# lizaibeim/mmla-audio

Hardware: AMD Instinct MI355X
Metric: audio clips/sec (MFCC→logits) at 1/2/4/8 MI355X; MFCC max-abs-err vs librosa (higher is better)
Workload: dtype f16x3+f32

## Files before the change

mmla_audio_amd/csrc/context.cpp:

```cpp
#include <algorithm>
#include <cstdarg>
#include <cstdio>
#include <cstdlib>

#include "internal.h"

using namespace mmla;

namespace mmla __attribute__((visibility("hidden"))) {

int fail(mmla_ctx* c, int code, const char* fmt, ...) {
  char buf[512];
  va_list ap;
  va_start(ap, fmt);
  vsnprintf(buf, sizeof(buf), fmt, ap);
  va_end(ap);
  if (c) c->err = buf;
  return code;
}

static hipEvent_t prof_event(mmla_ctx* c) {
  if (!c->prof_pool.empty()) {
    hipEvent_t e = c->prof_pool.back();
    c->prof_pool.pop_back();
// ... 77 lines not shown
  return MMLA_OK;
}

int ws_release(mmla_ctx* c) {
  HIPCHK(c, hipStreamSynchronize(c->stream));
  for (size_t i = 0; i < c->ws.size(); ++i)
    if (c->ws[i]) {
      HIPCHK(c, hipFree(static_cast<char*>(c->ws[i]) - c->ws_guard[i]));
      c->ws[i] = nullptr;
      c->ws_size[i] = 0;
      c->ws_guard[i] = 0;
    }
  return MMLA_OK;
}

static int ws_check_guards(mmla_ctx* c) {
  std::vector<unsigned char> h(kGuardBytes);
  for (size_t slot = 0; slot < c->ws.size(); ++slot) {
    const size_t g = c->ws_guard[slot];
    if (!c->ws[slot] || !g) continue;
    for (int side = 0; side < 2; ++side) {
      const char* d = static_cast<const char*>(c->ws[slot]) + (side ? c->ws_size[slot] : -(ptrdiff_t)g);
      HIPCHK(c, hipMemcpy(h.data(), d, g, hipMemcpyDeviceToHost));
      for (size_t i = 0; i < g; ++i)
        if (h[i] != kGuardByte)
          return fail(c, MMLA_E_HIP, "workspace slot %zu: %s guard overwritten at byte %zu", slot,
                      side ? "trailing" : "leading", side ? i : g - i);
    }
  }
  return MMLA_OK;
}

int finish(mmla_ctx* c, bool dev) {
  HIPCHK(c, hipGetLastError());
  bool guarded = false;
  for (size_t g : c->ws_guard) guarded |= g != 0;
  if (!dev || guarded) HIPCHK(c, hipStreamSynchronize(c->stream));
  if (guarded) return ws_check_guards(c);
  return MMLA_OK;
}

constexpr double kOdBytesPerClip = 3.0 * 128 * 151 * 32 * 4 + 128 * 151 * 3 + 128 * 151 * 4 +
                                   19 * 128 * 4 + 512 * 4 + 64;
constexpr double kSiBytesPerClip = 4.0 * 256 * 32 * 4 + 256 * 39 * 4 + 8 * 128 * 4 + 512 * 4 +
                                   1024 * 4 + 64;

int64_t microbatch(mmla_ctx* c, bool od) {
  const int64_t user = od ? c->od_mb : c->si_mb;
  if (user > 0) return user;
  const int64_t cap = od ? c->od_mb_cap : c->si_mb_cap;
  size_t fr = 0, tot = 0;
  if (hipMemGetInfo(&fr, &tot) != hipSuccess) {
    (void)hipGetLastError();
    return cap;
  }
  double held = 0;
  for (size_t b : c->ws_size) held += (double)b;
  int64_t fit = (int64_t)(((double)fr + held) * 0.9 / (od ? kOdBytesPerClip : kSiBytesPerClip));
  fit = fit / kMinMicrobatch * kMinMicrobatch;
  return std::max(kMinMicrobatch, std::min(cap, fit));
}

}

struct EnvSwitch {
  const char* name;
  bool mmla_ctx::*no;
  int mmla_ctx::*num;
};
static const EnvSwitch kEnvSwitches[] = {
    {"MMLA_DEBUG_FAIL_ALLOC", nullptr, &mmla_ctx::debug_fail_allocs},
    {"MMLA_NO_SIU", &mmla_ctx::siu, nullptr},
    {"MMLA_NO_SIPU", &mmla_ctx::sipu, nullptr},
    {"MMLA_NO_SIFIN", &mmla_ctx::sifin, nullptr},
    {"MMLA_NO_SIPAIR", &mmla_ctx::sipair, nullptr},
    {"MMLA_NO_SICHAIN", &mmla_ctx::sichain, nullptr},
    {"MMLA_NO_LSTM_SPLIT", &mmla_ctx::lstm_split, nullptr},
    {"MMLA_LSTM_SPLIT_MAX", nullptr, &mmla_ctx::lstm_split_max},
    {"MMLA_DEBUG_LSTM_SPIN", nullptr, &mmla_ctx::lstm_spin},
    {"MMLA_NO_SIPAD", &mmla_ctx::si_pad_feat, nullptr},
    {"MMLA_NO_ODU", &mmla_ctx::odu, nullptr},
    {"MMLA_NO_ODW", &mmla_ctx::odw, nullptr},
    {"MMLA_RB_TILE", &mmla_ctx::rbs, nullptr},
    {"MMLA_NO_PIN_OUT", &mmla_ctx::pin_small, nullptr},
};

extern "C" {

int mmla_abi_version(void) { return MMLA_ABI_VERSION; }

int mmla_create(int device, mmla_ctx** out) {
  if (!out) return MMLA_E_INVALID;
  *out = nullptr;
  int ndev = 0;
  if (hipGetDeviceCount(&ndev) != hipSuccess || ndev == 0) return MMLA_E_HIP;
  if (device < 0 || device >= ndev) return MMLA_E_INVALID;
  if (hipSetDevice(device) != hipSuccess) return MMLA_E_HIP;
  mmla_ctx* c = new mmla_ctx();
  c->device = device;
  for (const EnvSwitch& s : kEnvSwitches)
    if (const char* v = std::getenv(s.name)) {
      if (s.no) c->*s.no = std::atoi(v) == 0;
      else c->*s.num = std::atoi(v);
    }
  if (hipStreamCreateWithFlags(&c->own_stream, hipStreamDefault) != hipSuccess) {
    delete c;
    return MMLA_E_HIP;
  }
  c->stream = c->own_stream;
  if (hipMalloc(&c->range_dev, 4 * sizeof(int)) != hipSuccess ||
      hipMemset(c->range_dev, 0, 4 * sizeof(int)) != hipSuccess ||
      hipHostMalloc(&c->range_host, 2 * sizeof(int), hipHostMallocDefault) != hipSuccess) {
    mmla_destroy(c);
    return MMLA_E_HIP;
  }
  if (c->pin_small) {
    const unsigned fl = hipHostMallocMapped | hipHostMallocCoherent;
    if (hipHostMalloc(reinterpret_cast<void**>(&c->range_map), 64, fl) != hipSuccess ||
        hipHostGetDevicePointer(reinterpret_cast<void**>(&c->range_map_dev), c->range_map, 0) != hipSuccess ||
        hipHostMalloc(reinterpret_cast<void**>(&c->pin_out), kPinSlots * kPinSlotBytes, fl) != hipSuccess ||
        hipHostGetDevicePointer(reinterpret_cast<void**>(&c->pin_out_dev), c->pin_out, 0) != hipSuccess ||
        hipHostMalloc(reinterpret_cast<void**>(&c->pin_in), kPinInBytes, hipHostMallocDefault) != hipSuccess) {
      mmla_destroy(c);
      return MMLA_E_HIP;
    }
    c->range_map[0] = c->range_map[1] = 0;
  }
  OdFeTables ot;
  od_fe_build_tables(&ot);
  if (!od_fe_tables_ok(ot)) {
    mmla_destroy(c);
    return MMLA_E_INVALID;
  }
  SiFeTables st;
  si_fe_build_tables(&st);
  if (!si_fe_tables_ok(st)) {
    mmla_destroy(c);
    return MMLA_E_INVALID;
  }
  if (hipMalloc(&c->od_tables, sizeof(OdFeTables)) != hipSuccess ||
      hipMalloc(&c->si_tables, sizeof(SiFeTables)) != hipSuccess ||
      hipMemcpy(c->od_tables, &ot, sizeof(ot), hipMemcpyHostToDevice) != hipSuccess ||
      hipMemcpy(c->si_tables, &st, sizeof(st), hipMemcpyHostToDevice) != hipSuccess) {
    mmla_destroy(c);
    return MMLA_E_HIP;
  }
  *out = c;
  return MMLA_OK;
}

int mmla_destroy(mmla_ctx* c) {
  if (!c) return MMLA_E_INVALID;
  (void)hipSetDevice(c->device);
  if (c->stream) (void)hipStreamSynchronize(c->stream);
  free_allocs(c->od_allocs);
  free_allocs(c->si_allocs);
  for (size_t i = 0; i < c->ws.size(); ++i)
    if (c->ws[i]) (void)hipFree(static_cast<char*>(c->ws[i]) - c->ws_guard[i]);
  if (c->od_tables) (void)hipFree(c->od_tables);
  if (c->si_tables) (void)hipFree(c->si_tables);
  if (c->nr_tables) (void)hipFree(c->nr_tables);
  if (c->nr_thresh) (void)hipFree(c->nr_thresh);
  if (c->range_dev) (void)hipFree(c->range_dev);
  if (c->vad_state) (void)hipFree(c->vad_state);
  if (c->range_host) (void)hipHostFree(c->range_host);
  if (c->range_map) (void)hipHostFree(c->range_map);
// ... 120 lines not shown
```

mmla_audio_amd/csrc/internal.h:

```cpp
#pragma once
#include <hip/hip_runtime.h>

#include <cstdint>
#include <cstring>
#include <string>
#include <vector>

#include "../../include/mmla.h"
#include "nr.h"
#include "od_fe.h"
#include "si_fe.h"
#include "ssim.h"
#include "vad.h"

namespace mmla __attribute__((visibility("hidden"))) {

constexpr int OD_H = 128, OD_W = 151, OD_PIX = OD_H * OD_W;
constexpr int OD_IMG = OD_PIX * 3;
constexpr int SI_T = 256, SI_D = 39;
constexpr int SI_NEED_SAMPLES = 160 * 259 + 400;
constexpr int CH[9] = {32, 32, 32, 64, 64, 64, 128, 128, 128};
constexpr bool POOL[9] = {true, false, false, true, false, false, true, false, false};

struct ConvW {
// ... 8 lines not shown
  float unscale() const { return 1.0f / (16.0f * wscale); }
};
struct BnW {
  float* scale = nullptr;
  float* shift = nullptr;
  int c = 0;
};
struct LstmW {
  float* wcat[2] = {nullptr, nullptr};
  float* bias[2] = {nullptr, nullptr};
  uint16_t* wth[2] = {nullptr, nullptr};
  uint16_t* wtl[2] = {nullptr, nullptr};
  float ws[2] = {256.0f, 256.0f};
};
struct ResUnitW {
  BnW bn_in, bn_mid;
  ConvW ca, cb, sc;
};
struct OdNet {
  ConvW stem;
  ResUnitW blk[9];
  LstmW lstm;
  float* head_w = nullptr;
  float* head_b = nullptr;
};
struct SiNet {
  ConvW stem;
  ResUnitW unit[9];
  BnW final_bn;
  LstmW lstm;
  ConvW dense;
  int k = 0, head = 0;
};

struct ProfRec {
  int stage;
  hipEvent_t a, b;
  double work;
};

constexpr int64_t kOdMicrobatch = 16384;
constexpr int64_t kSiMicrobatch = 65536;
constexpr int64_t kMinMicrobatch = 64;

constexpr size_t kPinSlotBytes = 64u << 10;
constexpr size_t kPinInBytes = 1u << 20;
constexpr int kPinSlots = 4;

}

struct mmla_ctx {
  bool prof_on = false;
  std::vector<mmla::ProfRec> prof_pending;
  std::vector<hipEvent_t> prof_pool;
  double prof_ms[MMLA_NSTAGES] = {0};
  double prof_work[MMLA_NSTAGES] = {0};
  int64_t prof_n[MMLA_NSTAGES] = {0};
  int device = 0;
  hipStream_t stream = nullptr;
  hipStream_t own_stream = nullptr;
  std::string err;
  OdFeTables* od_tables = nullptr;
  SiFeTables* si_tables = nullptr;
  bool od_loaded = false, si_loaded = false;
  mmla::OdNet od;
  mmla::SiNet si;
  std::vector<void*> od_allocs, si_allocs;
  std::vector<void*> ws;
  std::vector<size_t> ws_size;
  std::vector<size_t> ws_guard;
  int64_t od_mb = 0, si_mb = 0;
  int64_t od_mb_cap = mmla::kOdMicrobatch, si_mb_cap = mmla::kSiMicrobatch;
  int debug_fail_allocs = 0;
  int precision = MMLA_PREC_F16X3;
  bool siu = true;
  bool sipu = true;
  bool sifin = true;
  bool sipair = true;
  bool sichain = true;
  bool si_pad_feat = true;
  bool odu = true;
  bool odw = true;
  bool rbs = true;
  bool lstm_split = true;
  int lstm_split_max = 128;
  int lstm_spin = 0;
  int* range_dev = nullptr;
  int* range_host = nullptr;
  bool pin_small = true;
  int* range_map = nullptr;
  int* range_map_dev = nullptr;
  char* pin_out = nullptr;
  char* pin_out_dev = nullptr;
  char* pin_in = nullptr;
  int* range_ptr = nullptr;
  int* timeout_ptr = nullptr;
  int64_t lstm_split_reruns = 0;
  int64_t range_reruns = 0;
  bool od_f32_only = false, si_f32_only = false;
  bool loading_f16_bad = false;
  VadState* vad_state = nullptr;
  int64_t vad_streams = 0;
  NrTables* nr_tables = nullptr;
  float* nr_thresh = nullptr;
  int64_t nr_profiles = 0;
  bool nr_ready = false;
};

namespace mmla __attribute__((visibility("hidden"))) {

int fail(mmla_ctx* c, int code, const char* fmt, ...);

#define HIPCHK(ctx, expr)                                                                        \
  do {                                                                                           \
    hipError_t e_ = (expr);                                                                      \
    if (e_ != hipSuccess)                                                                        \
      return mmla::fail(ctx, MMLA_E_HIP, "%s failed: %s (%s:%d)", #expr, hipGetErrorString(e_), \
                        __FILE__, __LINE__);                                                     \
  } while (0)

#define CHK(expr)              \
  do {                         \
    int r_ = (expr);           \
    if (r_ != MMLA_OK) return r_; \
  } while (0)

int prof_begin(mmla_ctx* c, int stage);
void prof_end(mmla_ctx* c, int idx, double work);
int prof_collect(mmla_ctx* c);

#define LAUNCH(c, st, wk, expr)                  \
  do {                                           \
    const int pi_ = mmla::prof_begin((c), (st)); \
    HIPCHK((c), (expr));                         \
    mmla::prof_end((c), pi_, (wk));              \
  } while (0)

enum Slot {
  S_PCM = 0, S_LENS, S_IMG, S_X, S_T1, S_T2, S_T3, S_SEQ, S_HOUT, S_LOGIT, S_FEAT, S_SILENT,
  S_OUT0, S_OUT1, S_OUT2, S_OUT3, S_IN,
  S_NR_S, S_NR_BITS, S_NR_FMAX, S_NR_FRAMES, S_NR_ITEMS, S_NR_Y, S_NR_ROWS,
  S_VAD_SPEECH, S_VAD_OUT, S_VAD_LENS, S_RS_TR, S_RS_WIN, S_LSTM,
  S_TRAIN,
  S_IMG2, S_GATE_Y0, S_GATE_Y1, S_SSIM,
  S_NR_PROF, S_COND_Q, S_COND_KEPT
};

int ws_get(mmla_ctx* c, int slot, size_t bytes, void** out);
int ws_release(mmla_ctx* c);
int64_t microbatch(mmla_ctx* c, bool od);
int finish(mmla_ctx* c, bool dev);
void free_allocs(std::vector<void*>& al);
int nr_reduce_dev(mmla_ctx* c, const float* y, int64_t n_signals, int64_t stride, int64_t len, float* out,
                  const int32_t* profile = nullptr);

template <typename T>
int in_ptr(mmla_ctx* c, const T* user, size_t count, bool dev, int slot, const T** d) {
  *d = user;
  if (dev || !user) return MMLA_OK;
  void* p = nullptr;
  CHK(ws_get(c, slot, count * sizeof(T), &p));
  HIPCHK(c, hipMemcpyAsync(p, user, count * sizeof(T), hipMemcpyHostToDevice, c->stream));
  *d = static_cast<const T*>(p);
  return MMLA_OK;
}

// ... 51 lines not shown
```

mmla_audio_amd/csrc/net_runners.cpp:

```cpp
#include <algorithm>

#include "conv.h"
#include "conv_h3.h"
#include "internal.h"
#include "nets.h"
#include "odu.h"
#include "resblk.h"
#include "siu.h"

using namespace mmla;

namespace {

ConvArgs conv_args(const ConvW& w, const float* x, float* y, int n, int h, int wd, int stride,
                   const BnW* bn, int pro, int epi, const float* res) {
  ConvArgs a{};
  a.x = x;
  a.wt = w.wt;
  a.bias = w.bias;
  a.scale = bn ? bn->scale : nullptr;
  a.shift = bn ? bn->shift : nullptr;
  a.res = res;
  a.y = y;
  a.n = n;
// ... 208 lines not shown
  o.s_in = B.bn_in.scale;
  o.t_in = B.bn_in.shift;
  o.s_mid = B.bn_mid.scale;
  o.t_mid = B.bn_mid.shift;
  o.ua = B.ca.unscale();
  o.ub = B.cb.unscale();
  o.n = (int)n;
  o.range_flag = range_flag;
  if (pool) {
    o.wsh = B.sc.wh;
    o.wsl = B.sc.wl;
    o.bs = B.sc.bias;
    o.us = B.sc.unscale();
  }
  return o;
}

double od_block_flops(const ResUnitW& B, bool pool, int64_t n, int h, int w) {
  return 2.0 * n * h * w * (9.0 * B.ca.cin * B.ca.cout + 4.0 * B.cb.cin * B.cb.cout) +
         (pool ? 2.0 * n * ((h + 1) / 2) * ((w + 1) / 2) * B.sc.cin * B.sc.cout : 0.0);
}

int od_block_pair(mmla_ctx* c, const ResUnitW& B, bool pool, int n, int h, int w, float* X, float*& T1,
                  float*& T2, float** out) {
  CHK(conv_spatial(c, B.ca, X, T1, n, h, w, &B.bn_in, PRO_BN_ELU, EPI_BIAS, nullptr));
  if (!pool) {
    *out = X;
    return conv_spatial(c, B.cb, T1, X, n, h, w, &B.bn_mid, PRO_BN_ELU, EPI_ADD, X);
  }
  if (c->precision != MMLA_PREC_F16X3) {
    CHK(conv_spatial(c, B.cb, T1, T2, n, h, w, &B.bn_mid, PRO_BN_ELU, EPI_BIAS, nullptr));
    ConvArgs s = conv_args(B.sc, X, T1, n, h, w, 2, nullptr, PRO_NONE, EPI_ADD_POOL, T2);
    s.hp = h;
    s.wp = w;
    CHK(conv_run(c, s));
  } else if (B.sc.wh && B.sc.cout == B.cb.cout && B.cb.cout_pad == B.sc.cout_pad) {
    CHK(conv_spatial(c, B.cb, T1, T2, n, h, w, &B.bn_mid, PRO_BN_ELU, EPI_BIAS, nullptr, true, 0, &B.sc,
                     X));
    std::swap(T1, T2);
  } else {
    CHK(conv_spatial(c, B.cb, T1, T2, n, h, w, &B.bn_mid, PRO_BN_ELU, EPI_BIAS, nullptr, true));
    CHK(conv_run(c, conv_args(B.sc, X, T1, n, h, w, 2, nullptr, PRO_NONE, EPI_ADD, T2)));
  }
  *out = T1;
  return MMLA_OK;
}

}

namespace mmla __attribute__((visibility("hidden"))) {

int run_od_net(mmla_ctx* c, const uint8_t* img_u8, const float* img_f32, int64_t n, float* probs,
               int32_t* argmax, OdGate gate, int stop, const float** tap, int64_t* tap_n) {
  const OdNet& W = c->od;
  const size_t big = (size_t)n * OD_PIX * 32;
  float *X, *T1, *T2, *SEQ, *H;
  CHK(ws_floats(c, S_X, big, &X));
  CHK(ws_floats(c, S_T1, big, &T1));
  CHK(ws_floats(c, S_T2, big, &T2));
  CHK(ws_floats(c, S_SEQ, (size_t)n * 19 * 128, &SEQ));
  CHK(ws_floats(c, S_HOUT, (size_t)n * 512, &H));
  const double stem_flops = 2.0 * n * OD_PIX * 3 * 16;
  const OdChoice first = od_choose(c, W.blk[0], 0, OD_H, OD_W, stop);
  if (!first.stem)
    LAUNCH(c, MMLA_STAGE_GLUE, stem_flops,
           od_stem_launch(img_u8, img_f32, n * OD_PIX, W.stem.cout_pad, W.stem.wt, W.stem.bias, X,
                          c->stream));
  int h = OD_H, w = OD_W;
  if (stop == 0) {
    *tap = X;
    *tap_n = n * OD_PIX * 16;
    return MMLA_OK;
  }
  for (int b = 0; b < 9; ++b) {
    const ResUnitW& B = W.blk[b];
    const bool pool = POOL[b];
    const OdChoice k = b == 0 ? first : od_choose(c, B, b, h, w, stop);
    const double flops = od_block_flops(B, pool, n, h, w) + (k.stem ? stem_flops : 0.0);
    float* out = T1;
    switch (k.path) {
      case OD_STRIPS:
      case OD_TILES: {
        const bool tiles = k.path == OD_TILES;
        const ResBlkArgs r = resblk_args(B, pool, tiles, X, T1, n, h, w, c->range_ptr,
                                         k.stem ? &W.stem : nullptr, img_u8, img_f32);
        LAUNCH(c, MMLA_STAGE_CONV, flops,
               tiles ? resblk_launch(r, B.ca.cin, B.ca.cout, pool, c->stream)
                     : rbs_launch(r, B.ca.cin, B.ca.cout, pool, c->stream));
        break;
      }
      case OD_ODU: {
        const OduArgs o = odu_args(B, pool, X, T1, n, c->range_ptr);
        LAUNCH(c, MMLA_STAGE_CONV, flops,
               odu_launch(o, h, w, B.ca.cin, B.ca.cout, pool, k.strips, c->stream));
        break;
      }
      case OD_PAIR:
        CHK(od_block_pair(c, B, pool, (int)n, h, w, X, T1, T2, &out));
        break;
    }
    if (pool) {
      h = (h + 1) / 2;
      w = (w + 1) / 2;
    }
    if (out != X) std::swap(X, T1);
    if (stop == b + 1) {
      *tap = X;
      *tap_n = n * h * w * CH[b];
      return MMLA_OK;
    }
  }
  LAUNCH(c, MMLA_STAGE_GLUE, (double)n * h * w * 128,
         mean_h_launch(X, (int)n, h, w, 128, SEQ, c->stream));
  if (stop == 10) {
    *tap = SEQ;
    *tap_n = n * w * 128;
    return MMLA_OK;
  }
  LAUNCH(c, MMLA_STAGE_LSTM, lstm_flops(n, w, 128),
         lstm_run(c, W.lstm, SEQ, n, w, H));
  if (stop == 11) {
    *tap = H;
    *tap_n = n * 512;
    return MMLA_OK;
  }
  LAUNCH(c, MMLA_STAGE_HEAD, 2.0 * n * 512 * 2,
         od_head_launch(H, (int)n, W.head_w, W.head_b, probs, argmax,
                        gate.lens, gate.clip_len, gate.silent, gate.ssim, gate.ssim_threshold,
                        c->stream));
  return MMLA_OK;
}

}


namespace {

bool siu_ok(const ResUnitW& U, int cin) {
  return U.ca.wh && U.cb.wh && siu_supported(cin) && U.ca.cin == cin && U.ca.cout == cin && U.cb.cin == cin &&
         U.cb.cout == cin && U.ca.cin_pad == cin && U.ca.cout_pad == cin && U.cb.cout_pad == cin;
}

bool sipu_ok(const ResUnitW& U, int cin) {
  return U.ca.wh && U.cb.wh && U.sc.wh && sipu_supported(cin, U.ca.cout) && U.ca.cin_pad == cin &&
         U.ca.cout_pad == U.ca.cout && U.cb.cin == U.ca.cout && U.cb.cout == U.ca.cout &&
         U.cb.cout_pad == U.ca.cout && U.sc.cin == cin && U.sc.cout == U.ca.cout &&
         U.sc.cout_pad == U.ca.cout;
}

SiuArgs siu_args(const ResUnitW& U, const float* x, float* y, int64_t n, int t, int* range_flag,
                 int t_src = 0) {
  SiuArgs s{};
  s.n = (int)n;
  s.t = t;
  s.range_flag = range_flag;
  s.x = x;
  s.y = y;
  s.wah = U.ca.wh;
  s.wal = U.ca.wl;
  s.wbh = U.cb.wh;
  s.wbl = U.cb.wl;
  s.ba = U.ca.bias;
  s.bb = U.cb.bias;
  s.s_in = U.bn_in.scale;
  s.t_in = U.bn_in.shift;
  s.s_mid = U.bn_mid.scale;
  s.t_mid = U.bn_mid.shift;
  s.ua = U.ca.unscale();
// ... 130 lines not shown
```

mmla_audio_amd/csrc/rbs.hip:

```cpp
#include "f16x3.h"
#include "resblk.h"

namespace {

constexpr int NT = 256;
constexpr int TW = 16;
constexpr int R = 8;
constexpr int C = 32;
#ifndef RBS_TRACE
#define RBS_TRACE 0
#endif
#if RBS_TRACE
__device__ unsigned long long rbs_trace_buf[2048 * 4 * 4 * 8];
#define RBS_T(i) do { if (bid < 2048 && k >= 2 && k < 6) tt[i] = __builtin_amdgcn_s_memtime(); } while (0)
#define RBS_TFLUSH() do { if (bid < 2048 && k >= 2 && k < 6 && lane == 0) { for (int i_ = 0; i_ < 8; ++i_) rbs_trace_buf[(((size_t)bid * 4 + wave) * 4 + (k - 2)) * 8 + i_] = tt[i_]; } } while (0)
#else
#define RBS_T(i) do { } while (0)
#define RBS_TFLUSH() do { } while (0)
#endif

template <int H, int W, int CIN, bool POOL>
struct SG {
  static constexpr int XW = TW + 2;
  static constexpr int XRING = R + 2, TRING = R + 3;
  static constexpr int XROW = XW * CIN;
  static constexpr int XPLANE = XRING * XROW;
  static constexpr int TROW = TW * C;
  static constexpr int TPLANE = TRING * TROW;
  static constexpr int NCHUNK = H / R;
  static constexpr int STRIPS = (W + TW - 1) / TW;
  static constexpr int QPP = CIN / 4;
  static constexpr int MAXT = (R * XW * QPP + NT - 1) / NT;
  static constexpr int MAXT0 = (4 * XW * QPP + NT - 1) / NT;
  static constexpr int KPT = CIN / 16;
  static constexpr int KS1 = 9 * KPT, KS2 = 8;
  static constexpr bool W2L = CIN == 16;
  static constexpr int MINB = CIN == 16 ? 3 : 2;
  static constexpr int PF = 3;
  static constexpr int PD = CIN == 16 ? 1 : 2;
  static_assert(H % R == 0, "geometry");
  static_assert(NT % QPP == 0, "a thread's channel quad is fixed");
  static_assert(XROW <= 1024 && W * CIN * 4 < 65536 && W * 12 < 65536, "staging task fields");
};

template <int CIN>
MMLA_DEV int xoff(int slot, int x, int g) {
  constexpr int XROW = (TW + 2) * CIN;
  const int f = CIN == 32 ? ((x >> 1) & 3) : ((x >> 1) & 1);
  return slot * XROW + x * CIN + 8 * (g ^ f);
}
template <bool POOL>
MMLA_DEV int toff(int slot, int j, int c, int g) {
  const int f = POOL ? (((c >> 2) ^ (2 * (j & 1))) & 3) : ((c >> 2) & 3);
  return slot * (TW * C) + c * C + 8 * (g ^ f);
}

template <int H, int W, int CIN, bool POOL, bool STEM>
__global__ void __launch_bounds__(NT, (SG<H, W, CIN, POOL>::MINB)) rbs_kernel(ResBlkArgs a) {
  using G = SG<H, W, CIN, POOL>;
  static_assert(!STEM || (CIN == 16 && POOL), "the stem feeds block 1");
  static_assert(POOL || CIN == C, "residual blocks keep their width");
  __shared__ __attribute__((aligned(16))) _Float16 sx[2 * G::XPLANE];
  __shared__ __attribute__((aligned(16))) _Float16 st[2 * G::TPLANE];
  __shared__ float4 spar[3 * C / 4 + (STEM ? 16 : 0)];
  __shared__ __attribute__((aligned(16))) _Float16 sw2[G::W2L ? 2 * G::KS2 * 512 : 8];

  const int tid = threadIdx.x, lane = tid & 63;
  const int wave = __builtin_amdgcn_readfirstlane(tid >> 6);
  const int h = lane >> 5;
  const uint32_t bid = xcd_block_id();
  const int clip = (int)(bid / G::STRIPS);
  const int w0 = (int)(bid - (uint32_t)clip * G::STRIPS) * TW;
  const int lofs = lane * 8;
  float rmax = 0.0f;

  float* const sp = reinterpret_cast<float*>(spar);
  if (tid < C) {
    const float s2 = a.s2[tid];
    sp[tid] = 16.0f * (s2 * a.u1);
    sp[C + tid] = 16.0f * fmaf(a.b1[tid], s2, a.t2[tid]);
    sp[2 * C + tid] = a.b2[tid];
  }
  if constexpr (STEM) {
    if (tid < 64) {
      const int co = tid >> 2, k = tid & 3;
      sp[3 * C + tid] = k < 3 ? a.wst[k * a.ldst + co] : a.bst[co];
    }
  }
  const __amdgpu_buffer_rsrc_t rw1h = w_rsrc(a.w1h), rw1l = w_rsrc(a.w1l);
  f16x8 w2h[G::W2L ? 1 : G::KS2], w2l[G::W2L ? 1 : G::KS2];
  if constexpr (G::W2L) {
    for (int e = tid; e < 2 * G::KS2 * 64; e += NT) {
      const int pl = e / (G::KS2 * 64), i = e - pl * (G::KS2 * 64);
      *reinterpret_cast<f16x8*>(sw2 + 8 * e) = *reinterpret_cast<const f16x8*>((pl ? a.w2l : a.w2h) + 8 * i);
    }
  } else {
    const __amdgpu_buffer_rsrc_t rw2h = w_rsrc(a.w2h), rw2l = w_rsrc(a.w2l);
#pragma unroll
    for (int s = 0; s < G::KS2; ++s) {
      w2h[s] = w_frag(rw2h, s * 512, lofs);
      w2l[s] = w_frag(rw2l, s * 512, lofs);
    }
  }
  f16x8 wsh_, wsl_;
  if constexpr (POOL) {
    wsh_ = w_frag(w_rsrc(a.wsh), 0, lofs);
    wsl_ = w_frag(w_rsrc(a.wsl), 0, lofs);
  }
  const int q = tid % G::QPP;
  float bnw[4][4];
  __syncthreads();
#pragma unroll
  for (int c = 0; c < 4; ++c) {
    const float s16 = 16.0f * a.s1[4 * q + c], t16 = 16.0f * a.t1[4 * q + c];
    if constexpr (STEM) {
      const float4 v = spar[3 * C / 4 + 4 * q + c];
      bnw[c][0] = s16 * v.x;
      bnw[c][1] = s16 * v.y;
      bnw[c][2] = s16 * v.z;
      bnw[c][3] = fmaf(s16, v.w, t16);
    } else {
      bnw[c][0] = s16;
      bnw[c][1] = t16;
    }
  }

  constexpr uint32_t ROWB = STEM ? 0u : (uint32_t)W * CIN * 4;
  const __amdgpu_buffer_rsrc_t rx = STEM ? w_rsrc(nullptr) :
      __builtin_amdgcn_make_buffer_rsrc(const_cast<float*>(a.x) + (int64_t)clip * H * W * CIN, (short)0,
                                        (int)(H * ROWB), 0x00020000);
  const bool im8 = STEM && a.img8 != nullptr;
  const __amdgpu_buffer_rsrc_t rimg = !STEM ? w_rsrc(nullptr) :
      __builtin_amdgcn_make_buffer_rsrc(im8 ? (void*)(a.img8 + (int64_t)clip * H * W * 3)
                                            : (void*)(a.imgf + (int64_t)clip * H * W * 3),
                                        (short)0, (int)(H * W * 3 * (im8 ? 1 : 4)), 0x00020000);
  uint32_t tinfo[G::MAXT];
#pragma unroll
  for (int j = 0; j < G::MAXT; ++j) {
    const int t = tid + j * NT;
    const int px = t / G::QPP;
    const int rr = px / G::XW, x = px - rr * G::XW;
    const int iw = w0 - 1 + x;
    const bool col_ok = iw >= 0 && iw < W;
    const uint32_t tc = !col_ok ? 0u : STEM ? (uint32_t)iw * (a.img8 ? 3u : 12u) : (uint32_t)(iw * CIN + 4 * q) * 4u;
    tinfo[j] = (uint32_t)(xoff<CIN>(0, x, q >> 1) + 4 * (q & 1)) | ((uint32_t)(rr & 15) << 10) |
               ((uint32_t)col_ok << 14) | ((uint32_t)(rr < R) << 15) | (tc << 16);
  }
  auto load_src = [&](int ih, int iw, bool col_ok) -> float4 {
    if constexpr (STEM) {
      const int pix = ih * W + iw;
      const bool ok = col_ok && ih >= 0 && ih < H;
      if (im8) {
        const uint32_t off = ok ? (uint32_t)pix * 3u : 0x80000000u;
        const uint32_t r = __builtin_amdgcn_raw_buffer_load_b8(rimg, off, 0, 0);
        const uint32_t g = __builtin_amdgcn_raw_buffer_load_b8(rimg, off + 1u, 0, 0);
        const uint32_t b = __builtin_amdgcn_raw_buffer_load_b8(rimg, off + 2u, 0, 0);
        return make_float4(__builtin_bit_cast(float, r), __builtin_bit_cast(float, g), __builtin_bit_cast(float, b), 0.f);
      }
      const uint32_t off = ok ? (uint32_t)pix * 12u : 0x80000000u;
      return make_float4(__builtin_bit_cast(float, __builtin_amdgcn_raw_buffer_load_b32(rimg, off, 0, 0)),
                         __builtin_bit_cast(float, __builtin_amdgcn_raw_buffer_load_b32(rimg, off + 4u, 0, 0)),
                         __builtin_bit_cast(float, __builtin_amdgcn_raw_buffer_load_b32(rimg, off + 8u, 0, 0)), 0.f);
    } else {
      const uint32_t off = col_ok ? (uint32_t)ih * ROWB + (uint32_t)(iw * CIN + 4 * q) * 4u : 0x80000000u;
      return __builtin_bit_cast(float4, __builtin_amdgcn_raw_buffer_load_b128(rx, off, 0, 0));
    }
  };
  auto img_px = [&](float4 v) -> float4 {
    if (im8)
      return make_float4((float)__builtin_bit_cast(uint32_t, v.x), (float)__builtin_bit_cast(uint32_t, v.y),
                         (float)__builtin_bit_cast(uint32_t, v.z), 0.f);
    return v;
  };
  auto load_task = [&](int r0, int j) -> float4 {
    const uint32_t ti = tinfo[j];
    const uint32_t off = (ti >> 14) & 1u ? (uint32_t)((r0 + (int)((ti >> 10) & 15)) * (STEM ? W * 3 * (im8 ? 1 : 4) : (int)ROWB)) + (ti >> 16)
                                         : 0x80000000u;
    if constexpr (STEM) {
      if (im8) {
        const uint32_t r = __builtin_amdgcn_raw_buffer_load_b8(rimg, off, 0, 0);
        const uint32_t g = __builtin_amdgcn_raw_buffer_load_b8(rimg, off + 1u, 0, 0);
        const uint32_t b = __builtin_amdgcn_raw_buffer_load_b8(rimg, off + 2u, 0, 0);
        return make_float4(__builtin_bit_cast(float, r), __builtin_bit_cast(float, g), __builtin_bit_cast(float, b), 0.f);
      }
      return make_float4(__builtin_bit_cast(float, __builtin_amdgcn_raw_buffer_load_b32(rimg, off, 0, 0)),
                         __builtin_bit_cast(float, __builtin_amdgcn_raw_buffer_load_b32(rimg, off + 4u, 0, 0)),
                         __builtin_bit_cast(float, __builtin_amdgcn_raw_buffer_load_b32(rimg, off + 8u, 0, 0)), 0.f);
    } else {
      return __builtin_bit_cast(float4, __builtin_amdgcn_raw_buffer_load_b128(rx, off, 0, 0));
    }
  };
  auto stage4 = [&](int o, bool in, float4 v, auto MASK_) {
    constexpr bool MASK = decltype(MASK_)::value;
    if constexpr (STEM) v = img_px(v);
    float u[4];
#pragma unroll
    for (int c = 0; c < 4; ++c) {
      if constexpr (STEM) {
        float acc = v.x * bnw[c][0];
        acc = fmaf(v.y, bnw[c][1], acc);
        acc = fmaf(v.z, bnw[c][2], acc);
        u[c] = acc + bnw[c][3];
      } else {
        u[c] = fmaf((&v.x)[c], bnw[c][0], bnw[c][1]);
      }
    }
    float e[4];
#pragma unroll
    for (int c = 0; c < 4; ++c) e[c] = (!MASK || in) ? elu16(u[c]) : 0.0f;
    rmax = fmaxf(rmax, amax4(e[0], e[1], e[2], e[3]));
    f16x4 hv, lv;
    split4(e[0], e[1], e[2], e[3], hv, lv);
    *reinterpret_cast<f16x4*>(sx + o) = hv;
    *reinterpret_cast<f16x4*>(sx + G::XPLANE + o) = lv;
  };
  auto stage_task = [&](int r0, int j, float4 v, auto MASK_) {
    const uint32_t ti = tinfo[j];
    if (((ti >> 14) & 3u) != 3u) return;
    const int rr = (int)((ti >> 10) & 15);
    uint32_t slot = (uint32_t)((r0 + 1) % G::XRING) + (uint32_t)rr;
    slot = min(slot, slot - (uint32_t)G::XRING);
    stage4((int)slot * G::XROW + (int)(ti & 1023), r0 + rr < H, v, MASK_);
  };
  for (int e = tid; e < 2 * G::XRING * G::XW * G::QPP; e += NT) {
    const int pl = e / (G::XRING * G::XW * G::QPP), r = e - pl * (G::XRING * G::XW * G::QPP);
    const int slot = r / (G::XW * G::QPP), x = (r / G::QPP) % G::XW, qq = r % G::QPP;
    const int iw = w0 - 1 + x;
    if (iw < 0 || iw >= W)
      *reinterpret_cast<f16x4*>(sx + pl * G::XPLANE + xoff<CIN>(slot, x, qq >> 1) + 4 * (qq & 1)) = f16x4{};
  }
  const int n = lane & 31, nr = n >> 4, nc = n & 15;
  int xco[3][G::KPT];
#pragma unroll
  for (int dx = 0; dx < 3; ++dx)
#pragma unroll
    for (int ks = 0; ks < G::KPT; ++ks) xco[dx][ks] = xoff<CIN>(0, nc + dx, G::KPT == 2 ? 2 * ks + h : h);

  f16x8 w1h[G::PF], w1l[G::PF];
  auto gemm1_issue = [&]() {
#pragma unroll
    for (int s = 0; s < G::PF; ++s) {
      w1h[s] = w_frag(rw1h, s * 512, lofs);
      w1l[s] = w_frag(rw1l, s * 512, lofs);
    }
  };
  auto gemm1 = [&](int j0) -> f32x16 {
    f32x16 acc;
#pragma unroll
    for (int i = 0; i < 16; ++i) acc[i] = 0.0f;
    int xr[3];
#pragma unroll
    for (int dy = 0; dy < 3; ++dy) {
      const uint32_t sl = (uint32_t)(j0 % G::XRING) + (uint32_t)(nr + dy);
      xr[dy] = (int)min(sl, sl - (uint32_t)G::XRING) * G::XROW;
    }
    auto xo = [&](int s) {
      const int tap = s / G::KPT, ks = s % G::KPT;
      return xr[tap / 3] + xco[tap % 3][ks];
    };
    f16x8 nxh = *reinterpret_cast<const f16x8*>(sx + xo(0));
    f16x8 nxl = *reinterpret_cast<const f16x8*>(sx + G::XPLANE + xo(0));
#pragma unroll
    for (int s = 0; s < G::KS1; ++s) {
      const f16x8 bh = w1h[s % G::PF], bl = w1l[s % G::PF];
      if (s + G::PF < G::KS1) {
        w1h[s % G::PF] = w_frag(rw1h, (s + G::PF) * 512, lofs);
        w1l[s % G::PF] = w_frag(rw1l, (s + G::PF) * 512, lofs);
      }
      const f16x8 xh = nxh, xl = nxl;
      if (s + 1 < G::KS1) {
        nxh = *reinterpret_cast<const f16x8*>(sx + xo(s + 1));
        nxl = *reinterpret_cast<const f16x8*>(sx + G::XPLANE + xo(s + 1));
      }
      acc = __builtin_amdgcn_mfma_f32_32x32x16_f16(bl, xh, acc, 0, 0, 0);
      acc = __builtin_amdgcn_mfma_f32_32x32x16_f16(bh, xl, acc, 0, 0, 0);
      acc = __builtin_amdgcn_mfma_f32_32x32x16_f16(bh, xh, acc, 0, 0, 0);
      __builtin_amdgcn_sched_barrier(0);
    }
    return acc;
  };
  auto t1_write = [&](int j0, const f32x16& acc) {
    const int j = j0 + nr;
    const uint32_t sl = (uint32_t)((j0 + 1) % G::TRING) + (uint32_t)nr;
    const int slot = (int)min(sl, sl - (uint32_t)G::TRING);
    if (j0 < H) {
#pragma unroll
      for (int jj = 0; jj < 4; ++jj) {
        const int c0 = 8 * jj + 4 * h;
        const float4 sv = spar[c0 / 4], cv = spar[C / 4 + c0 / 4];
        float e[4];
        e[0] = elu16(fmaf(acc[4 * jj + 0], sv.x, cv.x));
        e[1] = elu16(fmaf(acc[4 * jj + 1], sv.y, cv.y));
        e[2] = elu16(fmaf(acc[4 * jj + 2], sv.z, cv.z));
        e[3] = elu16(fmaf(acc[4 * jj + 3], sv.w, cv.w));
        rmax = fmaxf(rmax, amax4(e[0], e[1], e[2], e[3]));
        f16x4 hv, lv;
        split4(e[0], e[1], e[2], e[3], hv, lv);
        const int o = toff<POOL>(slot, j, nc, jj) + 4 * h;
        *reinterpret_cast<f16x4*>(st + o) = hv;
        *reinterpret_cast<f16x4*>(st + G::TPLANE + o) = lv;
      }
    } else {
#pragma unroll
      for (int jj = 0; jj < 4; ++jj) {
        const int o = toff<POOL>(slot, j, nc, jj) + 4 * h;
        *reinterpret_cast<f16x4*>(st + o) = f16x4{};
        *reinterpret_cast<f16x4*>(st + G::TPLANE + o) = f16x4{};
      }
    }
  };

  {
    constexpr int T0 = 4 * G::XW * G::QPP;
#pragma unroll
    for (int j = 0; j < G::MAXT0; ++j) {
      const int t = tid + j * NT;
      const int px = t / G::QPP;
      const int rr = px / G::XW, x = px - rr * G::XW;
      const int ih = rr - 1, iw = w0 - 1 + x;
      const bool col_ok = iw >= 0 && iw < W;
      const float4 v = load_src(ih, iw, col_ok);
      if (t < T0 && col_ok)
        stage4(xoff<CIN>((ih + 1) % G::XRING, x, q >> 1) + 4 * (q & 1), ih >= 0, v, std::true_type{});
    }
    for (int e = tid; e < 2 * G::TROW / 8; e += NT)
      *reinterpret_cast<f16x8*>(st + (e >= G::TROW / 8 ? G::TPLANE - G::TROW : 0) + 8 * e) = f16x8{};
  }
  __syncthreads();
  if (wave == 0) {
    gemm1_issue();
    const f32x16 acc = gemm1(0);
    t1_write(0, acc);
  }
  float4 preA[G::MAXT], preB[G::PD == 2 ? G::MAXT : 1];
#pragma unroll
  for (int j = 0; j < G::MAXT; ++j) preA[j] = load_task(3, j);
  if constexpr (G::PD == 2) {
#pragma unroll
    for (int j = 0; j < G::MAXT; ++j) preB[j] = load_task(3 + R, j);
  }
  __syncthreads();

  const int win = n >> 2;
  const int sc_col = w0 + 2 * win;
  float bsc = 0.0f;
  if constexpr (POOL) bsc = a.bs[n];

#if RBS_TRACE
  unsigned long long tt[8];
#endif
  static_assert(G::NCHUNK % 2 == 0, "chunk pairs");
  auto chunk = [&](const int k, float4* pre) {
    RBS_T(0);
    const int rx0 = R * k + 3;
    const int j0 = R * k + 2 + 2 * wave;
    const int o0 = R * k + 2 * wave;
    if (k + 1 < G::NCHUNK) {
#pragma unroll
      for (int j = 0; j < G::MAXT; ++j) stage_task(rx0, j, pre[j], std::false_type{});
    } else {
#pragma unroll
      for (int j = 0; j < G::MAXT; ++j) stage_task(rx0, j, pre[j], std::true_type{});
    }
    gemm1_issue();
    RBS_T(1);
    __syncthreads();
    RBS_T(2);
    {
      const f32x16 acc = gemm1(j0);
      RBS_T(3);
      t1_write(j0, acc);
    }
    RBS_T(4);
    const int pr = POOL ? (n & 3) >> 1 : nr;
    const int pc = POOL ? 2 * (n >> 2) + (n & 1) : nc;
    float4 rsd[POOL ? 1 : 4];
    float4 scpx = make_float4(0.f, 0.f, 0.f, 0.f);
    if constexpr (!POOL) {
      const uint32_t off = w0 + pc < W ? (uint32_t)(o0 + pr) * ROWB + (uint32_t)((w0 + pc) * C + 4 * h) * 4u : 0x80000000u;
#pragma unroll
      for (int jj = 0; jj < 4; ++jj)
        rsd[jj] = __builtin_bit_cast(float4, __builtin_amdgcn_raw_buffer_load_b128(rx, off, jj * 32, 0));
    } else {
      scpx = load_src(o0, sc_col, sc_col < W);
    }
    if (k + G::PD < G::NCHUNK) {
#pragma unroll
      for (int j = 0; j < G::MAXT; ++j) pre[j] = load_task(rx0 + G::PD * R, j);
    }
    __syncthreads();
    RBS_T(5);
    f32x16 acc;
#pragma unroll
    for (int i = 0; i < 16; ++i) acc[i] = 0.0f;
    {
      int tr[4], tj[4];
#pragma unroll
      for (int dy = 0; dy < 4; ++dy) {
        tj[dy] = o0 + pr - 1 + dy;
        const uint32_t sl = (uint32_t)(o0 % G::TRING) + (uint32_t)(pr + dy);
        tr[dy] = (int)min(sl, sl - (uint32_t)G::TRING);
      }
      auto to = [&](int s) { return toff<POOL>(tr[s >> 1], tj[s >> 1], pc, 2 * (s & 1) + h); };
      auto step2 = [&](f16x8 xh, f16x8 xl, f16x8 gh, f16x8 gl) {
        if constexpr (POOL) {
          acc = __builtin_amdgcn_mfma_f32_32x32x16_f16(xh, gl, acc, 0, 0, 0);
          acc = __builtin_amdgcn_mfma_f32_32x32x16_f16(xl, gh, acc, 0, 0, 0);
          acc = __builtin_amdgcn_mfma_f32_32x32x16_f16(xh, gh, acc, 0, 0, 0);
        } else {
          acc = __builtin_amdgcn_mfma_f32_32x32x16_f16(gl, xh, acc, 0, 0, 0);
          acc = __builtin_amdgcn_mfma_f32_32x32x16_f16(gh, xl, acc, 0, 0, 0);
          acc = __builtin_amdgcn_mfma_f32_32x32x16_f16(gh, xh, acc, 0, 0, 0);
        }
      };
      if constexpr (G::W2L) {
        f16x8 fxh[2], fxl[2], fgh[2], fgl[2];
        auto fetch = [&](int s) {
          fxh[s & 1] = *reinterpret_cast<const f16x8*>(st + to(s));
          fxl[s & 1] = *reinterpret_cast<const f16x8*>(st + G::TPLANE + to(s));
          fgh[s & 1] = *reinterpret_cast<const f16x8*>(sw2 + s * 512 + lofs);
          fgl[s & 1] = *reinterpret_cast<const f16x8*>(sw2 + (G::KS2 + s) * 512 + lofs);
        };
        fetch(0);
#pragma unroll
        for (int s = 0; s < G::KS2; ++s) {
          if (s + 1 < G::KS2) fetch(s + 1);
          step2(fxh[s & 1], fxl[s & 1], fgh[s & 1], fgl[s & 1]);
          if (s + 1 < G::KS2) pin_group<1, 4>(); else pin_group<1, 0>();
        }
      } else {
        f16x8 nxh = *reinterpret_cast<const f16x8*>(st + to(0));
        f16x8 nxl = *reinterpret_cast<const f16x8*>(st + G::TPLANE + to(0));
#pragma unroll
        for (int s = 0; s < G::KS2; ++s) {
          const f16x8 xh = nxh, xl = nxl;
          if (s + 1 < G::KS2) {
            nxh = *reinterpret_cast<const f16x8*>(st + to(s + 1));
            nxl = *reinterpret_cast<const f16x8*>(st + G::TPLANE + to(s + 1));
          }
          step2(xh, xl, w2h[s], w2l[s]);
          __builtin_amdgcn_sched_barrier(0);
        }
      }
    }
    RBS_T(6);
    if constexpr (!POOL) {
      const int ow = w0 + pc, oh = o0 + pr;
      if (ow < W) {
#pragma unroll
        for (int jj = 0; jj < 4; ++jj) {
          const int c0 = 8 * jj + 4 * h;
          const float4 b = spar[2 * C / 4 + c0 / 4];
          const float4 r = rsd[jj];
          const float4 v = make_float4(fmaf(acc[4 * jj + 0], a.u2, b.x) + r.x, fmaf(acc[4 * jj + 1], a.u2, b.y) + r.y,
                                       fmaf(acc[4 * jj + 2], a.u2, b.z) + r.z, fmaf(acc[4 * jj + 3], a.u2, b.w) + r.w);
          *reinterpret_cast<float4*>(a.y + (((int64_t)clip * H + oh) * W + ow) * C + c0) = v;
        }
      }
    } else {
      f32x16 sacc;
#pragma unroll
      for (int i = 0; i < 16; ++i) sacc[i] = 0.0f;
      {
        float o8[8];
        const float4 px = img_px(scpx);
#pragma unroll
        for (int c = 0; c < 8; ++c) {
          const float4 wv = spar[3 * C / 4 + 8 * h + c];
          float s = px.x * wv.x;
          s = fmaf(px.y, wv.y, s);
          s = fmaf(px.z, wv.z, s);
          o8[c] = sc_col < W ? 16.0f * (s + wv.w) : 0.0f;
        }
        rmax = fmaxf(rmax, fmaxf(amax4(o8[0], o8[1], o8[2], o8[3]), amax4(o8[4], o8[5], o8[6], o8[7])));
        f16x4 h0, l0, h1, l1;
        split4(o8[0], o8[1], o8[2], o8[3], h0, l0);
        split4(o8[4], o8[5], o8[6], o8[7], h1, l1);
        const f16x8 ah = {h0[0], h0[1], h0[2], h0[3], h1[0], h1[1], h1[2], h1[3]};
        const f16x8 al = {l0[0], l0[1], l0[2], l0[3], l1[0], l1[1], l1[2], l1[3]};
        sacc = __builtin_amdgcn_mfma_f32_32x32x16_f16(ah, wsl_, sacc, 0, 0, 0);
        sacc = __builtin_amdgcn_mfma_f32_32x32x16_f16(al, wsh_, sacc, 0, 0, 0);
        sacc = __builtin_amdgcn_mfma_f32_32x32x16_f16(ah, wsh_, sacc, 0, 0, 0);
      }
      constexpr int HP = H / 2, WP = (W + 1) / 2;
      const int co = n;
      const float b2 = sp[2 * C + co], bs = bsc;
      const int prow = (R / 2) * k + wave;
#pragma unroll
      for (int jj = 0; jj < 4; ++jj) {
        const int wdw = 2 * jj + h;
        const int cc = w0 + 2 * wdw;
        if (cc >= W) continue;
        float m0 = fmaf(acc[4 * jj + 0], a.u2, b2);
        float m1 = fmaf(acc[4 * jj + 1], a.u2, b2);
        float m2 = fmaf(acc[4 * jj + 2], a.u2, b2);
        float m3 = fmaf(acc[4 * jj + 3], a.u2, b2);
        if (cc + 1 >= W) {
          m1 = m0;
          m3 = m2;
        }
        const float mx = fmaxf(fmaxf(m0, m1), fmaxf(m2, m3)) + fmaf(sacc[4 * jj], a.us, bs);
        a.y[(((int64_t)clip * HP + prow) * WP + (w0 >> 1) + wdw) * C + co] = mx;
      }
    }
    RBS_T(7);
    RBS_TFLUSH();
  };
  if constexpr (G::PD == 2) {
#pragma unroll 1
    for (int k = 0; k < G::NCHUNK; k += 2) {
      chunk(k, preA);
      chunk(k + 1, preB);
    }
  } else {
#pragma unroll 1
    for (int k = 0; k < G::NCHUNK; ++k) chunk(k, preA);
  }
  if (!(rmax < SPLIT_MAX) && a.range_flag) *a.range_flag = 1;
}

template <int H, int W, int CIN, bool POOL, bool STEM>
hipError_t launch(const ResBlkArgs& a, hipStream_t s) {
  using G = SG<H, W, CIN, POOL>;
  const int64_t blocks = (int64_t)a.n * G::STRIPS;
  if (blocks > 0x7fffffffLL) return hipErrorInvalidValue;
  hipLaunchKernelGGL((rbs_kernel<H, W, CIN, POOL, STEM>), dim3((unsigned)blocks), dim3(NT), 0, s, a);
  return hipGetLastError();
}

}

#if RBS_TRACE
extern "C" int mmla_debug_rbs_trace(unsigned long long* out) {
  return hipMemcpyFromSymbol(out, HIP_SYMBOL(rbs_trace_buf), sizeof(rbs_trace_buf)) == hipSuccess ? 0 : -2;
}
#endif

bool rbs_supported(int h, int w, int cin, int c, bool pool) {
  return c == 32 && ((h == 128 && w == 151 && cin == 16 && pool) || (h == 64 && w == 76 && cin == 32 && !pool));
}

hipError_t rbs_launch(const ResBlkArgs& a, int cin, int c, bool pool, hipStream_t s) {
  if (a.n == 0) return hipSuccess;
  if (!rbs_supported(a.h, a.w, cin, c, pool) || !a.y || !a.w1h || !a.w1l || !a.w2h || !a.w2l)
    return hipErrorInvalidValue;
  if (pool) {
    if (!a.wsh || !a.wsl || !a.bs) return hipErrorInvalidValue;
    if (a.img8 || a.imgf) return launch<128, 151, 16, true, true>(a, s);
    return hipErrorInvalidValue;
  }
  if (!a.x || a.x == a.y) return hipErrorInvalidValue;
  return launch<64, 76, 32, false, false>(a, s);
}
```

mmla_audio_amd/csrc/resblk.h:

```cpp
#pragma once
#include <hip/hip_runtime.h>
#include <stdint.h>

struct ResBlkArgs {
  const float* x;
  const uint16_t* w1h;
  const uint16_t* w1l;
  const float* b1;
  const float* s1;
  const float* t1;
  const uint16_t* w2h;
  const uint16_t* w2l;
  const float* b2;
  const float* s2;
  const float* t2;
  const uint16_t* wsh;
  const uint16_t* wsl;
  const float* bs;
  const uint8_t* img8;
  const float* imgf;
  const float* wst;
  const float* bst;
  int ldst;
  float* y;
  int n, h, w;
  int tiles_h, tiles_w;
  int* range_flag;
  float u1, u2, us;
};

int resblk_k1pad(int cin);
bool resblk_supported(int cin, int c, bool pool);
hipError_t resblk_launch(ResBlkArgs a, int cin, int c, bool pool, hipStream_t stream);
void resblk_split_weights(const float* w, int taps, int cin, int cout, int kpad, uint16_t* hi,
                          uint16_t* lo, bool frag, float wscale);

bool rbs_supported(int h, int w, int cin, int c, bool pool);
hipError_t rbs_launch(const ResBlkArgs& a, int cin, int c, bool pool, hipStream_t stream);
```

Before: 164,400.

## Add persistent-block mode to strip resblock kernel with cross-clip input prefetch

Lets the strip residual-block kernel loop over several clips per block, launching only enough blocks to fill the device. The next clip's prologue and first task rows are prefetched during the last chunks of the current clip. The aim is to hide per-clip prologue latency and block launch/tail costs. The mode is gated behind an env switch, but the restructured kernel body (hoisted prologue loads, extra buffer resources, extra VGPR-pinned values) runs in every case and may raise register pressure.

```diff
diff --git a/mmla_audio_amd/csrc/context.cpp b/mmla_audio_amd/csrc/context.cpp
--- a/mmla_audio_amd/csrc/context.cpp
+++ b/mmla_audio_amd/csrc/context.cpp
@@ -183,6 +183,8 @@
     {"MMLA_NO_ODU", &mmla_ctx::odu, nullptr},
     {"MMLA_NO_ODW", &mmla_ctx::odw, nullptr},
     {"MMLA_RB_TILE", &mmla_ctx::rbs, nullptr},
+    {"MMLA_NO_RBS_PERSIST", &mmla_ctx::rbs_persist, nullptr},
+    {"MMLA_RBS_CLIPS_IN_FLIGHT", nullptr, &mmla_ctx::rbs_inflight},
     {"MMLA_NO_PIN_OUT", &mmla_ctx::pin_small, nullptr},
 };
 
diff --git a/mmla_audio_amd/csrc/internal.h b/mmla_audio_amd/csrc/internal.h
--- a/mmla_audio_amd/csrc/internal.h
+++ b/mmla_audio_amd/csrc/internal.h
@@ -114,6 +114,8 @@
   bool odu = true;
   bool odw = true;
   bool rbs = true;
+  bool rbs_persist = false;
+  int rbs_inflight = 0;
   bool lstm_split = true;
   int lstm_split_max = 128;
   int lstm_spin = 0;
diff --git a/mmla_audio_amd/csrc/net_runners.cpp b/mmla_audio_amd/csrc/net_runners.cpp
--- a/mmla_audio_amd/csrc/net_runners.cpp
+++ b/mmla_audio_amd/csrc/net_runners.cpp
@@ -314,8 +314,9 @@
       case OD_STRIPS:
       case OD_TILES: {
         const bool tiles = k.path == OD_TILES;
-        const ResBlkArgs r = resblk_args(B, pool, tiles, X, T1, n, h, w, c->range_ptr,
-                                         k.stem ? &W.stem : nullptr, img_u8, img_f32);
+        ResBlkArgs r = resblk_args(B, pool, tiles, X, T1, n, h, w, c->range_ptr,
+                                   k.stem ? &W.stem : nullptr, img_u8, img_f32);
+        r.inflight = c->rbs_persist ? std::max(0, c->rbs_inflight) : -1;
         LAUNCH(c, MMLA_STAGE_CONV, flops,
                tiles ? resblk_launch(r, B.ca.cin, B.ca.cout, pool, c->stream)
                      : rbs_launch(r, B.ca.cin, B.ca.cout, pool, c->stream));
diff --git a/mmla_audio_amd/csrc/rbs.hip b/mmla_audio_amd/csrc/rbs.hip
--- a/mmla_audio_amd/csrc/rbs.hip
+++ b/mmla_audio_amd/csrc/rbs.hip
@@ -66,12 +66,16 @@
   __shared__ __attribute__((aligned(16))) _Float16 sw2[G::W2L ? 2 * G::KS2 * 512 : 8];
 
   const int tid = threadIdx.x, lane = tid & 63;
-  const int wave = __builtin_amdgcn_readfirstlane(tid >> 6);
+  const int wave0 = __builtin_amdgcn_readfirstlane(tid >> 6);
+  int wave = wave0;
   const int h = lane >> 5;
   const uint32_t bid = xcd_block_id();
-  const int clip = (int)(bid / G::STRIPS);
+  int clip = (int)(bid / G::STRIPS);
   const int w0 = (int)(bid - (uint32_t)clip * G::STRIPS) * TW;
   const int lofs = lane * 8;
+  int v_n = a.n, v_f = a.inflight;
+  uint32_t v_rf0 = (uint32_t)(uintptr_t)a.range_flag, v_rf1 = (uint32_t)((uintptr_t)a.range_flag >> 32);
+  asm volatile("" : "+v"(v_n), "+v"(v_f), "+v"(v_rf0), "+v"(v_rf1));
   float rmax = 0.0f;
 
   float* const sp = reinterpret_cast<float*>(spar);
@@ -126,14 +130,19 @@
   }
 
   constexpr uint32_t ROWB = STEM ? 0u : (uint32_t)W * CIN * 4;
-  const __amdgpu_buffer_rsrc_t rx = STEM ? w_rsrc(nullptr) :
-      __builtin_amdgcn_make_buffer_rsrc(const_cast<float*>(a.x) + (int64_t)clip * H * W * CIN, (short)0,
-                                        (int)(H * ROWB), 0x00020000);
   const bool im8 = STEM && a.img8 != nullptr;
-  const __amdgpu_buffer_rsrc_t rimg = !STEM ? w_rsrc(nullptr) :
-      __builtin_amdgcn_make_buffer_rsrc(im8 ? (void*)(a.img8 + (int64_t)clip * H * W * 3)
-                                            : (void*)(a.imgf + (int64_t)clip * H * W * 3),
-                                        (short)0, (int)(H * W * 3 * (im8 ? 1 : 4)), 0x00020000);
+  auto clip_rsrc = [&](int cl) -> __amdgpu_buffer_rsrc_t {
+    const bool ok = cl < __builtin_amdgcn_readfirstlane(v_n);
+    const int64_t c0 = ok ? cl : 0;
+    if constexpr (STEM)
+      return __builtin_amdgcn_make_buffer_rsrc(im8 ? (void*)(a.img8 + c0 * H * W * 3) : (void*)(a.imgf + c0 * H * W * 3),
+                                               (short)0, ok ? (int)(H * W * 3 * (im8 ? 1 : 4)) : 0, 0x00020000);
+    else
+      return __builtin_amdgcn_make_buffer_rsrc(const_cast<float*>(a.x) + c0 * H * W * CIN, (short)0,
+                                               ok ? (int)(H * ROWB) : 0, 0x00020000);
+  };
+  int nclip = clip + a.inflight;
+  __amdgpu_buffer_rsrc_t rcur = clip_rsrc(clip), rnxt = clip_rsrc(nclip);
   uint32_t tinfo[G::MAXT];
 #pragma unroll
   for (int j = 0; j < G::MAXT; ++j) {
@@ -146,7 +155,8 @@
     tinfo[j] = (uint32_t)(xoff<CIN>(0, x, q >> 1) + 4 * (q & 1)) | ((uint32_t)(rr & 15) << 10) |
                ((uint32_t)col_ok << 14) | ((uint32_t)(rr < R) << 15) | (tc << 16);
   }
-  auto load_src = [&](int ih, int iw, bool col_ok) -> float4 {
+  auto load_src = [&](__amdgpu_buffer_rsrc_t rs, int ih, int iw, bool col_ok) -> float4 {
+    const __amdgpu_buffer_rsrc_t rimg = rs, rx = rs;
     if constexpr (STEM) {
       const int pix = ih * W + iw;
       const bool ok = col_ok && ih >= 0 && ih < H;
@@ -172,7 +182,8 @@
                          (float)__builtin_bit_cast(uint32_t, v.z), 0.f);
     return v;
   };
-  auto load_task = [&](int r0, int j) -> float4 {
+  auto load_task = [&](__amdgpu_buffer_rsrc_t rs, int r0, int j) -> float4 {
+    const __amdgpu_buffer_rsrc_t rimg = rs, rx = rs;
     const uint32_t ti = tinfo[j];
     const uint32_t off = (ti >> 14) & 1u ? (uint32_t)((r0 + (int)((ti >> 10) & 15)) * (STEM ? W * 3 * (im8 ? 1 : 4) : (int)ROWB)) + (ti >> 16)
                                          : 0x80000000u;
@@ -310,36 +321,46 @@
     }
   };
 
-  {
+  auto load_pro = [&](__amdgpu_buffer_rsrc_t rs, int j) -> float4 {
+    const int px = (tid + j * NT) / G::QPP;
+    const int rr = px / G::XW, x = px - rr * G::XW;
+    const int iw = w0 - 1 + x;
+    return load_src(rs, rr - 1, iw, iw >= 0 && iw < W);
+  };
+  float4 pro[G::MAXT0], preA[G::MAXT], preB[G::PD == 2 ? G::MAXT : 1];
+#pragma unroll
+  for (int j = 0; j < G::MAXT0; ++j) pro[j] = load_pro(rcur, j);
+#pragma unroll
+  for (int j = 0; j < G::MAXT; ++j) preA[j] = load_task(rcur, 3, j);
+  if constexpr (G::PD == 2) {
+#pragma unroll
+    for (int j = 0; j < G::MAXT; ++j) preB[j] = load_task(rcur, 3 + R, j);
+  }
+  auto prologue = [&]() {
     constexpr int T0 = 4 * G::XW * G::QPP;
+    int tp = tid, z = 0;
+    asm volatile("" : "+v"(tp), "+s"(z));
+    const int qp = tp % G::QPP;
 #pragma unroll
     for (int j = 0; j < G::MAXT0; ++j) {
-      const int t = tid + j * NT;
+      const int t = tp + j * NT;
       const int px = t / G::QPP;
       const int rr = px / G::XW, x = px - rr * G::XW;
       const int ih = rr - 1, iw = w0 - 1 + x;
       const bool col_ok = iw >= 0 && iw < W;
-      const float4 v = load_src(ih, iw, col_ok);
       if (t < T0 && col_ok)
-        stage4(xoff<CIN>((ih + 1) % G::XRING, x, q >> 1) + 4 * (q & 1), ih >= 0, v, std::true_type{});
-    }
-    for (int e = tid; e < 2 * G::TROW / 8; e += NT)
+        stage4(xoff<CIN>((ih + 1) % G::XRING, x, qp >> 1) + 4 * (qp & 1), ih >= 0, pro[j], std::true_type{});
+    }
+    __syncthreads();
+    for (int e = tp; e < 2 * G::TROW / 8; e += NT)
       *reinterpret_cast<f16x8*>(st + (e >= G::TROW / 8 ? G::TPLANE - G::TROW : 0) + 8 * e) = f16x8{};
-  }
-  __syncthreads();
-  if (wave == 0) {
-    gemm1_issue();
-    const f32x16 acc = gemm1(0);
-    t1_write(0, acc);
-  }
-  float4 preA[G::MAXT], preB[G::PD == 2 ? G::MAXT : 1];
-#pragma unroll
-  for (int j = 0; j < G::MAXT; ++j) preA[j] = load_task(3, j);
-  if constexpr (G::PD == 2) {
-#pragma unroll
-    for (int j = 0; j < G::MAXT; ++j) preB[j] = load_task(3 + R, j);
-  }
-  __syncthreads();
+    if (wave == 0) {
+      gemm1_issue();
+      const f32x16 acc = gemm1(z);
+      t1_write(z, acc);
+    }
+    __syncthreads();
+  };
 
   const int win = n >> 2;
   const int sc_col = w0 + 2 * win;
@@ -350,6 +371,7 @@
   unsigned long long tt[8];
 #endif
   static_assert(G::NCHUNK % 2 == 0, "chunk pairs");
+  float* yclip = a.y;
   auto chunk = [&](const int k, float4* pre) {
     RBS_T(0);
     const int rx0 = R * k + 3;
@@ -380,13 +402,20 @@
       const uint32_t off = w0 + pc < W ? (uint32_t)(o0 + pr) * ROWB + (uint32_t)((w0 + pc) * C + 4 * h) * 4u : 0x80000000u;
 #pragma unroll
       for (int jj = 0; jj < 4; ++jj)
-        rsd[jj] = __builtin_bit_cast(float4, __builtin_amdgcn_raw_buffer_load_b128(rx, off, jj * 32, 0));
-    } else {
-      scpx = load_src(o0, sc_col, sc_col < W);
-    }
-    if (k + G::PD < G::NCHUNK) {
-#pragma unroll
-      for (int j = 0; j < G::MAXT; ++j) pre[j] = load_task(rx0 + G::PD * R, j);
+        rsd[jj] = __builtin_bit_cast(float4, __builtin_amdgcn_raw_buffer_load_b128(rcur, off, jj * 32, 0));
+    } else {
+      scpx = load_src(rcur, o0, sc_col, sc_col < W);
+    }
+    {
+      const bool nx = k + G::PD >= G::NCHUNK;
+      const __amdgpu_buffer_rsrc_t rs = nx ? rnxt : rcur;
+      const int r0 = rx0 + G::PD * R - (nx ? H : 0);
+      if (k + G::PD == G::NCHUNK) {
+#pragma unroll
+        for (int j = 0; j < G::MAXT0; ++j) pro[j] = load_pro(rnxt, j);
+      }
+#pragma unroll
+      for (int j = 0; j < G::MAXT; ++j) pre[j] = load_task(rs, r0, j);
     }
     __syncthreads();
     RBS_T(5);
@@ -454,7 +483,7 @@
           const float4 r = rsd[jj];
           const float4 v = make_float4(fmaf(acc[4 * jj + 0], a.u2, b.x) + r.x, fmaf(acc[4 * jj + 1], a.u2, b.y) + r.y,
                                        fmaf(acc[4 * jj + 2], a.u2, b.z) + r.z, fmaf(acc[4 * jj + 3], a.u2, b.w) + r.w);
-          *reinterpret_cast<float4*>(a.y + (((int64_t)clip * H + oh) * W + ow) * C + c0) = v;
+          *reinterpret_cast<float4*>(yclip + (uint32_t)((oh * W + ow) * C + c0)) = v;
         }
       }
     } else {
@@ -482,7 +511,7 @@
         sacc = __builtin_amdgcn_mfma_f32_32x32x16_f16(al, wsh_, sacc, 0, 0, 0);
         sacc = __builtin_amdgcn_mfma_f32_32x32x16_f16(ah, wsh_, sacc, 0, 0, 0);
       }
-      constexpr int HP = H / 2, WP = (W + 1) / 2;
+      constexpr int WP = (W + 1) / 2;
       const int co = n;
       const float b2 = sp[2 * C + co], bs = bsc;
       const int prow = (R / 2) * k + wave;
@@ -500,29 +529,49 @@
           m3 = m2;
         }
         const float mx = fmaxf(fmaxf(m0, m1), fmaxf(m2, m3)) + fmaf(sacc[4 * jj], a.us, bs);
-        a.y[(((int64_t)clip * HP + prow) * WP + (w0 >> 1) + wdw) * C + co] = mx;
+        yclip[(uint32_t)((prow * WP + (w0 >> 1) + wdw) * C + co)] = mx;
       }
     }
     RBS_T(7);
     RBS_TFLUSH();
   };
-  if constexpr (G::PD == 2) {
 #pragma unroll 1
-    for (int k = 0; k < G::NCHUNK; k += 2) {
-      chunk(k, preA);
-      chunk(k + 1, preB);
-    }
-  } else {
+  for (; clip < __builtin_amdgcn_readfirstlane(v_n); clip = nclip, nclip += __builtin_amdgcn_readfirstlane(v_f)) {
+    wave = wave0;
+    asm volatile("" : "+s"(wave));
+    yclip = a.y + (int64_t)clip * ((POOL ? ((H + 1) / 2) * ((W + 1) / 2) : H * W) * C);
+    prologue();
+    if constexpr (G::PD == 2) {
 #pragma unroll 1
-    for (int k = 0; k < G::NCHUNK; ++k) chunk(k, preA);
-  }
-  if (!(rmax < SPLIT_MAX) && a.range_flag) *a.range_flag = 1;
+      for (int k = 0; k < G::NCHUNK; k += 2) {
+        chunk(k, preA);
+        chunk(k + 1, preB);
+      }
+    } else {
+#pragma unroll 1
+      for (int k = 0; k < G::NCHUNK; ++k) chunk(k, preA);
+    }
+    rcur = rnxt;
+    rnxt = clip_rsrc(nclip + __builtin_amdgcn_readfirstlane(v_f));
+  }
+  int* const range_flag = reinterpret_cast<int*>((uintptr_t)v_rf0 | ((uintptr_t)v_rf1 << 32));
+  if (!(rmax < SPLIT_MAX) && range_flag) *range_flag = 1;
 }
 
 template <int H, int W, int CIN, bool POOL, bool STEM>
-hipError_t launch(const ResBlkArgs& a, hipStream_t s) {
+hipError_t launch(ResBlkArgs a, hipStream_t s) {
   using G = SG<H, W, CIN, POOL>;
-  const int64_t blocks = (int64_t)a.n * G::STRIPS;
+  static const int n_cu = [] {
+    int dev = 0, v = 0;
+    if (hipGetDevice(&dev) != hipSuccess ||
+        hipDeviceGetAttribute(&v, hipDeviceAttributeMultiprocessorCount, dev) != hipSuccess || v <= 0)
+      v = 256;
+    return v;
+  }();
+  int f = a.inflight < 0 ? a.n : std::min(a.n, std::max(1, n_cu * G::MINB / G::STRIPS));
+  if (a.inflight > 0) f = std::min(f, a.inflight);
+  a.inflight = f;
+  const int64_t blocks = (int64_t)f * G::STRIPS;
   if (blocks > 0x7fffffffLL) return hipErrorInvalidValue;
   hipLaunchKernelGGL((rbs_kernel<H, W, CIN, POOL, STEM>), dim3((unsigned)blocks), dim3(NT), 0, s, a);
   return hipGetLastError();
diff --git a/mmla_audio_amd/csrc/resblk.h b/mmla_audio_amd/csrc/resblk.h
--- a/mmla_audio_amd/csrc/resblk.h
+++ b/mmla_audio_amd/csrc/resblk.h
@@ -25,6 +25,7 @@
   float* y;
   int n, h, w;
   int tiles_h, tiles_w;
+  int inflight;
   int* range_flag;
   float u1, u2, us;
 };
```

New measurement: 164,300 (median of 2 runs). No clear change (-0.1%).
